# LeCAR-Lab/CoVO-MPC

Measured on AMD Instinct MI355X. Metric: mpc_control_steps_per_sec, higher is better.
Workload: dtype f32; 1 GPU; covo-online tracking_zigzag N=65536 H=32 lam=0.01 sigma=0.5 (teacher-forced on the recorded inputs -- noisy state, a_mean, key -- of this controller's own 300-step closed-loop episode, timed steps spread evenly over the episode; samples sharded 1x65536, one exchange of the 516-float rank records per step: collective); controller=covo-online, task=tracking_zigzag, N_global=65536, N_local=65536, H=32, pos_stats_info=False

## Files before the change

covo_mpc_amd/csrc/sigma_ns.hip:

```cpp
#include "covo_common.hpp"
#include <cstdlib>
#include <cstring>
#include "wave_reduce.hpp"
#include "chol_lds.hpp"
#include "eps_tiles.hpp"
#include "sym_stats.hpp"
#include "noise_gemm_body.hpp"

typedef double f64x4 __attribute__((ext_vector_type(4)));

#ifdef NS_EVAL_STAMPS
#define EV_STAMP(s, i) do { if (threadIdx.x == 0) (s)[SC_STAMPS + 96 + (i)] = (double)wall_clock64(); } while (0)
#else
#define EV_STAMP(s, i) do { } while (0)
#endif
#define EV_STAMP8(s, k, i) do { if ((k) == 8) EV_STAMP(s, 70 + (i)); } while (0)
constexpr int SN = COVO_NA;
constexpr int NS_SQUARINGS = 16;
constexpr double NS_CUT_MARGIN = 1.0 / 1024.0;
constexpr double NS_SQ_TOL = 1e-7;
constexpr double NS_SQ_TGUARD = 1e10;
constexpr int NS_ITERS = 12;
constexpr double NS_TOL2 = 1e-8;
constexpr int RITZ = 4;
// ... 55 lines not shown
}

template <int MI, int MJ>
struct TileBlock {
    double a[MI][8], b[MJ][8];
};
template <int COH, class F>
__device__ __forceinline__ void tile_col_load(double (&o)[8], const double *M, int col, int kq, int hi, int kk0, int kk1, F f)
{
#pragma unroll
    for (int kk = kk0; kk < kk1; ++kk) {
        const int k = 32 * kq + 4 * kk + hi;
        o[kk] = f(gld<COH>(M + (size_t)k * SN + col), k, col);
    }
}
template <int COH, int MI, int MJ, class F>
__device__ __forceinline__ void block_load(TileBlock<MI, MJ> &o, const double *At, const double *B, int bi, int bj, int lane, int kq, F f)
{
    const int lo = lane & 15, hi = lane >> 4;
    const int ca = 16 * MI * bi + lo, cb = 16 * MJ * bj + lo;
#pragma unroll
    for (int half = 0; half < 2; ++half) {
        tile_col_load<COH>(o.a[0], At, ca, kq, hi, 4 * half, 4 * half + 4, f);
        tile_col_load<COH>(o.b[0], B, cb, kq, hi, 4 * half, 4 * half + 4, f);
        __builtin_amdgcn_sched_barrier(0);
    }
#pragma unroll
    for (int t = 1; t < MI * MJ; ++t) {
        const int ia = t / MJ, ib = t % MJ;
        if (ib == 0) tile_col_load<COH>(o.a[ia], At, ca + 16 * ia, kq, hi, 0, 8, f);
        if (ia == 0) tile_col_load<COH>(o.b[ib], B, cb + 16 * ib, kq, hi, 0, 8, f);
        __builtin_amdgcn_sched_barrier(0);
    }
}
template <int MI, int MJ>
__device__ __forceinline__ void block_mma_reduce(const TileBlock<MI, MJ> &o, double (*red)[4][4][64], int wv, int lane, double (&v)[MI * MJ],
                                                 bool skip0 = false)
{
#pragma unroll
    for (int t = 0; t < MI * MJ; ++t) {
        if (t == 0 && skip0) continue;
        f64x4 acc = {0.0, 0.0, 0.0, 0.0};
#pragma unroll
        for (int kk = 0; kk < 8; ++kk) acc = __builtin_amdgcn_mfma_f64_16x16x4f64(o.a[t / MJ][kk], o.b[t % MJ][kk], acc, 0, 0, 0);
#pragma unroll
        for (int r = 0; r < 4; ++r) red[t][wv][r][lane] = acc[r];
        __builtin_amdgcn_sched_barrier(0);
    }
// ... 680 lines not shown
    ritz_picks<COH_NONE>(ns_xk(xb, k - 1) + (size_t)b * SN * SN, s, L);
    RitzIn in;
    ritz_load_matrix(in, Aall + (size_t)b * SN * SN, s, tid);
    ritz_load_inputs<COH_NONE>(in, s, tid);
    const double u = ritz_eval<COH_NONE>(in, ns_xk(xb, k) + (size_t)b * SN * SN, s, k, L);
    (void)ritz_decide(L, u, s, k, final, deflate);
}

__device__ __forceinline__ void ns_coef(double l, double &a, double &bq)
{
    const double rho = (l < 1.0 - 1e-9) ? 1.7320508075688772 * qm::rsq64_(1.0 + l + l * l) : 1.0;
    a = 1.5 * rho;
    bq = -0.5 * rho * rho * rho;
}

struct NsFirst {
    const double *X1, *u;
    double ya, yx, yi, yu, za, zi, zu;
    double a1, b1;
};
__device__ __forceinline__ NsFirst ns_first_setup(const double *X1, const double *s)
{
#pragma clang fp contract(off)
    NsFirst f;
    const double scale = s[SC_SCALE], delta = s[SC_DELTA], lo = s[SC_LO], gam = s[SC_GAM];
    const double alpha = s[SC_ALPHA], beta = s[SC_BETA], n0 = s[SC_N0], t1 = s[SC_SQN + 64 + 63];
    const double inv = 1.0 / scale, ib2 = 1.0 / (beta * beta), is2 = inv * inv;
    double l = sqrt(lo / scale), a0, b0;
    ns_coef(l, a0, b0);
    l = fmin(1.0, l * fma(b0 * l, l, a0));
    ns_coef(l, f.a1, f.b1);
    const double qx = n0 * ib2 * is2, qa = (2.0 * alpha * beta * ib2 + 2.0 * delta) * is2;
    const double qi = ((n0 / t1 - alpha * alpha) * ib2 + delta * delta) * is2, qu = gam * (2.0 * (1e-2 * inv) + gam);
    f.ya = fma(b0, qa, a0 * inv);
    f.yx = b0 * qx;
    f.yi = fma(b0, qi, a0 * delta * inv);
    f.yu = fma(b0, qu, a0 * gam);
    f.za = b0 * inv;
    f.zi = fma(b0, delta * inv, a0);
    f.zu = b0 * gam;
    f.X1 = X1;
    f.u = s + SC_U;
    return f;
}
struct LoadY1 {
    NsFirst f;
    __device__ __forceinline__ double operator()(double v, int r, int c) const
    {
#pragma clang fp contract(off)
        return fma(f.ya, v, fma(f.yx, f.X1[(size_t)r * SN + c], fma(f.yu * f.u[r], f.u[c], (r == c) ? f.yi : 0.0)));
    }
};
struct LoadZ1 {
    NsFirst f;
    __device__ __forceinline__ double operator()(double v, int r, int c) const
    {
#pragma clang fp contract(off)
        return fma(f.za, v, fma(f.zu * f.u[r], f.u[c], (r == c) ? f.zi : 0.0));
    }
};
template <int COH>
__device__ __forceinline__ void ns_coef_table(double *s)
{
    const double scale = s[SC_SCALE], lo = s[SC_LO];
    double l = sqrt(lo / scale);
    for (int k = 0; k < NS_ITERS; ++k) {
        double a, bq;
        ns_coef(l, a, bq);
        gst<COH>(s + SC_COEF + 2 * k, a);
        gst<COH>(s + SC_COEF + 2 * k + 1, bq);
        l = fmin(1.0, l * fma(bq * l, l, a));
    }
}

struct NsConvAsk {
// ... 6 lines not shown
    c.done = gld<COH>(s + SC_NS_DONE);
    c.e = (iter >= 2) ? gld<COH>(s + SC_ERR + (iter - 1) * 64 + lane) : 0.0;
    return c;
}
template <int COH>
__device__ __forceinline__ bool ns_converged(const NsConvAsk c, double *s, int iter, bool writer)
{
    if (c.done != 0.0) return true;
    if (iter >= 2 && wr::wave64_allsum(c.e) < NS_TOL2) {
        if (writer) gst<COH>(s + SC_NS_DONE, 1.0);
        return true;
    }
    return false;
}

__global__ __launch_bounds__(256) void ns_first_elem_kernel(const double *__restrict__ Aall, const double *__restrict__ X1all,
                                                            double *__restrict__ Yout, double *__restrict__ Ytout,
                                                            double *__restrict__ Zout, double *__restrict__ Ztout,
                                                            double *__restrict__ scall, int zbuf_out, int batch)
{
    int b, w;
    if (!ns_block(batch, b, w)) return;
    const int tid = threadIdx.x;
    double *s = scall + (size_t)b * SC_COUNT;
    if (w == 64) {
        if (tid == 0) ns_coef_table<COH_NONE>(s);
        return;
    }
    const size_t off = (size_t)b * SN * SN;
    const NsFirst f = ns_first_setup(X1all + off, s);
    if (w == 0 && tid == 0) {
        s[SC_ZBUF] = (double)zbuf_out;
        s[SC_ITERS] = 1.0;
    }
    const int ti = w >> 3, tj = w & 7;
    const int row = 16 * ti + (tid >> 4), col = 16 * tj + (tid & 15);
    const double av = Aall[off + (size_t)row * SN + col];
    store_both(Yout + off, Ytout + off, row, col, LoadY1{f}(av, row, col));
    store_both(Zout + off, Ztout + off, row, col, LoadZ1{f}(av, row, col));
}

template <int COH, int MI, int MJ>
__device__ __forceinline__ bool ns_T_block_body(const double *Y, const double *Zt, double *T, double *Tt, double *s, int iter, int w,
                                                double (*red)[4][4][64], double (*part)[4])
{
    const int tid = threadIdx.x, lane = tid & 63, wv = tid >> 6;
    constexpr int NJ = 8 / MJ;
    const int bi = w / NJ, bj = w % NJ;
    if (ns_batch_done<COH>(s, SC_NS_DONE)) return false;
    TileBlock<MI, MJ> ops;
    const NsConvAsk conv = ns_converged_ask<COH>(s, iter, lane);
    const double a = gld<COH>(s + SC_COEF + 2 * iter), bq = gld<COH>(s + SC_COEF + 2 * iter + 1);
    block_load<COH>(ops, Zt, Y, bi, bj, lane, wv, LoadPlain{});
    if (ns_converged<COH>(conv, s, iter, w == 0 && tid == 0)) return false;
// ... 131 lines not shown
    __syncthreads();
    return res;
}

__device__ __forceinline__ bool ns_persist_block(int nw, int batch, int &b, int &w, unsigned xcd0 = 0u)
{
    const unsigned slot = blockIdx.x >> 3, xcd = (blockIdx.x - xcd0) & 7u;
    b = (int)(slot / (unsigned)nw) * 8 + (int)xcd;
    w = (int)(slot % (unsigned)nw);
    return b < batch;
}
static inline dim3 ns_persist_grid(int nw, int batch) { return dim3(8 * nw * ((batch + 7) / 8)); }

struct NsBufs {
    double *Y[2], *Yt[2], *Z[2], *Zt[2], *T, *Tt;
    const double *A, *X1;
};

constexpr int NS_SQ_EVAL_WG = 8;
constexpr int NS_SQ_EVAL_WG_BATCH = 3;
template <int COH, int NEVAL>
__device__ __forceinline__ void ns_square_tail_pair_rest(const XBufs xb, double *scall, int w, unsigned xcc, double (*redp)[4][4][64],
                                                         double (*partp)[4])
{
    constexpr int NW = NS_SQ_PAIR_WG + NEVAL;
    unsigned *flags = reinterpret_cast<unsigned *>(scall + SC_FLAGS);
    unsigned phase = 1;
    for (int step = 1; step < NS_SQUARINGS; ++step) {
        if (!ns_square_pair_body<false, COH>(ns_xk(xb, step), ns_xk(xb, step + 1), scall, step, w, redp, partp)) return;
        ++phase;
        const bool gd = w == 0;
// ... 114 lines not shown
    scall += (size_t)b * SC_COUNT;
    const unsigned xcc = ns_xcc_id();
    if (w >= NS_SQ_PAIR_WG) {
        if constexpr (DYN) {
            RitzLds &L = *reinterpret_cast<RitzLds *>(dyn + 2 * 4 * 4 * 64 + 8);
            ns_square_evaluator<NEVAL, LEAN>(A + (size_t)b * SN * SN, xb, scall, w - NS_SQ_PAIR_WG, xcc, deflate, L);
        } else {
            __shared__ RitzLds L;
            ns_square_evaluator<NEVAL, LEAN>(A + (size_t)b * SN * SN, xb, scall, w - NS_SQ_PAIR_WG, xcc, deflate, L);
        }
        return;
    }
    if (w == 0) EV_STAMP(scall, 0);
    (void)ns_square_pair_body<true, COH_AGENT>(A + (size_t)b * SN * SN, ns_xk(xb, 1), scall, 0, w, redp, partp);
    int r = ns_flag_barrier<COH_AGENT>(reinterpret_cast<unsigned *>(scall + SC_FLAGS), 1u, w, NW, xcc, scall + SC_BARFAIL);
    if (r == 2 && force_agent) r = 1;
    if (w == 0 && threadIdx.x == 0) scall[SC_PROF + 5] = (double)r;
    if (r == 2) ns_square_tail_pair_rest<COH_XCD, NEVAL>(xb, scall, w, xcc, redp, partp);
    else if (r == 1) ns_square_tail_pair_rest<COH_AGENT, NEVAL>(xb, scall, w, xcc, redp, partp);
    if (w == 0) EV_STAMP(scall, 1);
}
template <int NEVAL>
__global__ __launch_bounds__(256) void ns_square_tail_pair_kernel(const double *A, const XBufs xb_all, double *scall, int batch,
                                                                  int force_agent, int deflate)
{
    ns_square_tail_pair_impl<NEVAL, false>(A, xb_all, scall, batch, force_agent, deflate);
}
__global__ __launch_bounds__(256, 3) void ns_square_tail_pair_lean_kernel(const double *A, const XBufs xb_all, double *scall, int batch,
                                                                          int force_agent, int deflate)
{
    ns_square_tail_pair_impl<NS_SQ_EVAL_WG_BATCH, true>(A, xb_all, scall, batch, force_agent, deflate);
}

constexpr int NS_PAIR_WG = 32;
template <int COH>
__device__ __forceinline__ void ns_iter_tail_pair_rest(const NsBufs &B, size_t off, double *scall, int iter_first, int w, unsigned xcc,
                                                       double (*redp)[4][4][64], double (*partp)[4], bool t_first)
{
    constexpr int iter_last = NS_ITERS - 1;
    unsigned *flags = reinterpret_cast<unsigned *>(scall + SC_FLAGS) + 64;
    unsigned phase = 1;
    for (int iter = iter_first; iter <= iter_last; ++iter) {
        const bool odd = (iter & 1) != 0;
        const double *Yi = (odd ? B.Y[1] : B.Y[0]) + off, *Yti = (odd ? B.Yt[1] : B.Yt[0]) + off;
        const double *Zi = (odd ? B.Z[1] : B.Z[0]) + off, *Zti = (odd ? B.Zt[1] : B.Zt[0]) + off;
        double *Yo = (odd ? B.Y[0] : B.Y[1]) + off, *Yto = (odd ? B.Yt[0] : B.Yt[1]) + off;
        double *Zo = (odd ? B.Z[0] : B.Z[1]) + off, *Zto = (odd ? B.Zt[0] : B.Zt[1]) + off;
        if (iter > iter_first || t_first) {
            if (!ns_T_block_body<COH, 2, 1>(Yi, Zti, B.T + off, B.Tt + off, scall, iter, w, redp, partp)) return;
            if (!ns_flag_barrier<COH>(flags, ++phase, w, NS_PAIR_WG, xcc, scall + SC_BARFAIL)) return;
        }
        (void)ns_YZ_block_body<COH, 2, 2>(Yti, Zi, B.T + off, B.Tt + off, Yo, Yto, Zo, Zto, scall, iter, odd ? 0 : 1, w, redp);
        if (iter < iter_last && !ns_flag_barrier<COH>(flags, ++phase, w, NS_PAIR_WG, xcc, scall + SC_BARFAIL)) return;
    }
}
template <int NWAVES>
__device__ void ns_logdetB_workgroup(const double *__restrict__ A, double *__restrict__ s, double *__restrict__ sm, double *__restrict__ red);
constexpr int NS_BATCH_TAIL_ITERS = 4;
__device__ __forceinline__ bool ns_wait_result(double *s)
{
    __shared__ int ready_ok;
    if (threadIdx.x == 0) {
        const long long t0 = wall_clock64();
        int good = 1;
        while (gld<COH_AGENT>(s + SC_READY) == 0.0) {
            __builtin_amdgcn_s_sleep(2);
            if (wall_clock64() - t0 > 20000000LL) {
                good = 0;
                gst<COH_AGENT>(s + SC_BARFAIL, 1.0);
                break;
            }
        }
        ready_ok = good;
    }
    __syncthreads();
    return ready_ok != 0;
}
template <bool EARLY_LOGDET>
__device__ __forceinline__ void ns_iter_tail_pair_impl(const double *A, const NsBufs B, double *scall, int batch, int force_agent, int merged,
                                                       double *ld_sm)
{
    constexpr int iter_first = EARLY_LOGDET ? 1 : NS_ITERS - NS_BATCH_TAIL_ITERS;
    double (*redp)[4][4][64] = reinterpret_cast<double (*)[4][4][64]>(ld_sm);
    __shared__ double partp[2][4];
    if (EARLY_LOGDET && blockIdx.x == 2) {
        if (merged && !ns_wait_result(scall)) return;
        ns_logdetB_workgroup<4>(A, scall, ld_sm, &partp[0][0]);
        return;
    }
    if (EARLY_LOGDET && blockIdx.x == (merged ? 3u : 1u)) {
        if (merged && !ns_wait_result(scall)) return;
        if (threadIdx.x == 0) {
            ns_coef_table<COH_AGENT>(scall);
            asm volatile("s_waitcnt vmcnt(0)" ::: "memory");
            gst<COH_AGENT>(scall + SC_BAR, 1.0);
        }
        return;
    }
    int b, w;
    if (!ns_persist_block(NS_PAIR_WG, batch, b, w, merged ? 1u : 0u)) return;
    const size_t off = (size_t)b * SN * SN;
    scall += (size_t)b * SC_COUNT;
    const unsigned xcc = ns_xcc_id();
    constexpr bool odd = (iter_first & 1) != 0;
    if (merged && !ns_wait_result(scall)) return;
    if (EARLY_LOGDET) {
        const NsFirst f = ns_first_setup(B.X1 + off, scall);
        const LoadY1 fy{f};
        const LoadZ1 fz{f};
        const int tid = threadIdx.x, lane = tid & 63, wv = tid >> 6, p = w >> 3, tj = w & 7;
        if (w == 0 && tid == 0) {
            gst<COH_AGENT>(scall + SC_ZBUF, 1.0);
            gst<COH_AGENT>(scall + SC_ITERS, 1.0);
        }
#pragma unroll
        for (int h = 0; h < 2; ++h) {
            const int row = 16 * (2 * p + h) + (lane >> 4) + 4 * wv, col = 16 * tj + (lane & 15);
            const double av = (B.A + off)[(size_t)row * SN + col];
            store_both<COH_AGENT>(B.Y[1] + off, B.Yt[1] + off, row, col, fy(av, row, col));
            store_both<COH_AGENT>(B.Z[1] + off, B.Zt[1] + off, row, col, fz(av, row, col));
        }
    } else if (!ns_T_block_body<COH_AGENT, 2, 1>((odd ? B.Y[1] : B.Y[0]) + off, (odd ? B.Zt[1] : B.Zt[0]) + off, B.T + off, B.Tt + off, scall,
                                          iter_first, w, redp, partp))
        return;
    int r = ns_flag_barrier<COH_AGENT>(reinterpret_cast<unsigned *>(scall + SC_FLAGS) + 64, 1u, w, NS_PAIR_WG, xcc, scall + SC_BARFAIL);
    if (r == 2 && force_agent) r = 1;
    if (w == 0 && threadIdx.x == 0) scall[SC_PROF + 6] = (double)r;
    if (EARLY_LOGDET) {
        __shared__ int tab_ok;
        if (threadIdx.x == 0) {
            const long long t0 = wall_clock64();
            int good = 1;
            while (gld<COH_AGENT>(scall + SC_BAR) == 0.0) {
                __builtin_amdgcn_s_sleep(1);
                if (wall_clock64() - t0 > 20000000LL) {
                    good = 0;
                    gst<COH_AGENT>(scall + SC_BARFAIL, 1.0);
                    break;
                }
            }
            tab_ok = good;
        }
        __syncthreads();
        if (!tab_ok) return;
    }
    if (r == 2) ns_iter_tail_pair_rest<COH_XCD>(B, off, scall, iter_first, w, xcc, redp, partp, EARLY_LOGDET);
    else if (r == 1) ns_iter_tail_pair_rest<COH_AGENT>(B, off, scall, iter_first, w, xcc, redp, partp, EARLY_LOGDET);
}
template <bool EARLY_LOGDET>
__global__ __launch_bounds__(256) void ns_iter_tail_pair_kernel(const double *A, const NsBufs B, double *scall, int batch, int force_agent)
{
    extern __shared__ __attribute__((aligned(16))) double ld_sm[];
    ns_iter_tail_pair_impl<EARLY_LOGDET>(A, B, scall, batch, force_agent, 0, ld_sm);
}
template <int NEVAL>
__global__ __launch_bounds__(256) void ns_chain_kernel(const double *A, const XBufs xb_all, const NsBufs B, double *scall, int force_agent,
                                                       int deflate)
{
    extern __shared__ __attribute__((aligned(16))) double ld_sm[];
    static_assert(NS_SQ_DYN_DOUBLES * sizeof(double) <= (size_t)SN * (SN + 1) * sizeof(double), "the squaring side's LDS fits the launch's");
    static_assert(NS_SQ_PAIR_WG + NEVAL <= NS_PAIR_WG, "grid = 8 x NS_PAIR_WG covers the squaring side");
    if ((blockIdx.x & 7u) == 0u) {
// ... 533 lines not shown
    double *sc = ws + (size_t)11 * batch * SN * SN;
    SymStatsOut o;
    o.rpart = sc + SC_RPART;
    o.fpart = sc + SC_FPART;
    o.diag = sc + SC_DIAG;
    o.stride = SC_COUNT;
    o.flags = sc + SC_FLAGS;
    o.ready = sc + SC_READY;
    return o;
}
const double *sigma_ns_sumlogB(void *workspace, int batch, size_t *stride_doubles)
{
    *stride_doubles = SC_COUNT;
    return reinterpret_cast<double *>(workspace) + (size_t)11 * batch * SN * SN + SC_SUMLOGB;
}
size_t sigma_ns_workspace_bytes(int batch) { return (size_t)batch * ((11 + NS_SQUARINGS - 1) * SN * SN + SC_COUNT) * sizeof(double); }

template <int MI, int MJ>
static void ns_launch_iters(hipStream_t s, const NsBufs &B, double *sc, int i_end, int batch)
{
    hipLaunchKernelGGL(ns_first_elem_kernel, ns_grid(65, batch), dim3(256), 0, s, B.A, B.X1, B.Y[1], B.Yt[1], B.Z[1], B.Zt[1], sc, 1, batch);
    for (int i = 1; i < i_end; ++i) {
        const int in = i & 1, out = in ^ 1;
        hipLaunchKernelGGL((ns_T_quad_kernel<MI, MJ>), ns_grid(64 / (MI * MJ), batch), dim3(256), 0, s, B.Y[in], B.Zt[in], B.T, B.Tt, sc, i,
                           batch);
        hipLaunchKernelGGL((ns_YZ_quad_kernel<MI, MJ>), ns_grid(128 / (MI * MJ), batch), dim3(256), 0, s, B.Yt[in], B.Z[in], B.T, B.Tt,
                           B.Y[out], B.Yt[out], B.Z[out], B.Zt[out], sc, i, out, batch);
    }
}

int launch_sigma_ns(const CovoOpts &opt, const SigmaNsDesc &d, void *workspace, hipStream_t s, const DebugMasks &dbg)
{
    const double *R = d.R;
    const int batch = d.batch;
    const float sample_sigma = d.sample_sigma;
    float *Sigma = d.Sigma;
    CovDeferred *cov = d.cov;
// ... 20 lines not shown
        COVO_CHECK_HIP(hipFuncSetAttribute(reinterpret_cast<const void *>(ns_finalize_stream_kernel),
                                           hipFuncAttributeMaxDynamicSharedMemorySize, (int)lds));
    }
    if (d.r_has_stats) A = const_cast<double *>(R);
    else hipLaunchKernelGGL(ns_prep_kernel, ns_grid(NS_TILES, batch), dim3(256), 0, s, R, A, sc, batch);
    NsBufs B;
    for (int k = 0; k < 2; ++k) {
        B.Y[k] = Y[k];
        B.Yt[k] = Yt[k];
        B.Z[k] = Z[k];
        B.Zt[k] = Zt[k];
    }
    B.T = hist0;
    B.Tt = hist0 + M;
    B.A = A;
    B.X1 = ns_xk(xb, 1);
    enum { MERGED, TWO_LAUNCH, BATCHED, PHASED } plan;
    if (!d.persistent_ok) plan = PHASED;
    else if (batch > 1) plan = BATCHED;
    else if (opt.ns_merged && d.r_has_stats && sigma_stages >= 3) plan = MERGED;
    else plan = TWO_LAUNCH;
    switch (plan) {
    case MERGED:
        hipLaunchKernelGGL((ns_chain_kernel<NS_SQ_EVAL_WG>), ns_persist_grid(NS_PAIR_WG, 1), dim3(256), lds, s, A, xb, B, sc, opt.ns_force_agent,
                           opt.ns_deflate);
        break;
    case TWO_LAUNCH:
        hipLaunchKernelGGL((ns_square_tail_pair_kernel<NS_SQ_EVAL_WG>), ns_persist_grid(NS_SQ_PAIR_WG + NS_SQ_EVAL_WG, 1), dim3(256), 0, s, A,
                           xb, sc, 1, opt.ns_force_agent, opt.ns_deflate);
        if (sigma_stages < 3) return 0;
        hipLaunchKernelGGL(ns_iter_tail_pair_kernel<true>, ns_persist_grid(NS_PAIR_WG, 1), dim3(256), lds, s, A, B, sc, 1, opt.ns_force_agent);
        break;
    case BATCHED:
        hipLaunchKernelGGL(ns_square_tail_pair_lean_kernel, ns_persist_grid(NS_SQ_PAIR_WG + NS_SQ_EVAL_WG_BATCH, batch), dim3(256), 0, s, A,
                           xb, sc, batch, opt.ns_force_agent, opt.ns_deflate);
        if (sigma_stages < 3) return 0;
        ns_launch_iters<2, 2>(s, B, sc, NS_ITERS - NS_BATCH_TAIL_ITERS, batch);
        hipLaunchKernelGGL(ns_iter_tail_pair_kernel<false>, ns_persist_grid(NS_PAIR_WG, batch), dim3(256), 4 * 4 * 4 * 64 * sizeof(double), s, A,
                           B, sc, batch, opt.ns_force_agent);
        break;
    case PHASED:
        if (batch == 1) {
            hipLaunchKernelGGL((ns_square_kernel<true, 1>), ns_grid(NS_TILES, 1), dim3(256), 0, s, A, ns_xk(xb, 1), sc, 0, 1);
            for (int i = 1; i < NS_SQUARINGS; ++i)
                hipLaunchKernelGGL((ns_square_kernel<false, 1>), ns_grid(NS_TILES, 1), dim3(256), 0, s, ns_xk(xb, i), ns_xk(xb, i + 1), sc, i, 1);
        } else {
            hipLaunchKernelGGL((ns_square_kernel<true, 2>), ns_grid(NS_SQ_PAIR_WG, batch), dim3(256), 0, s, A, ns_xk(xb, 1), sc, 0, batch);
            for (int i = 1; i < NS_SQUARINGS; ++i)
                hipLaunchKernelGGL((ns_square_kernel<false, 2>), ns_grid(NS_SQ_PAIR_WG, batch), dim3(256), 0, s, ns_xk(xb, i), ns_xk(xb, i + 1),
                                   sc, i, batch);
        }
        if (sigma_stages < 2) return 0;
        hipLaunchKernelGGL(ns_ritz_scan_kernel, dim3(batch * RITZ_NK), dim3(256), 0, s, A, xb, sc, opt.ns_deflate);
        if (sigma_stages < 3) return 0;
        if (batch == 1) ns_launch_iters<1, 1>(s, B, sc, NS_ITERS, batch);
        else ns_launch_iters<2, 2>(s, B, sc, NS_ITERS, batch);
        break;
    }
    if (sigma_stages < 4) return 0;
    const bool early_logdet = plan == MERGED || plan == TWO_LAUNCH;
    if (stream != nullptr && early_logdet) {
        const int ntiles = (stream->N + 31) / 32;
        const int workers = (ntiles - 8 + 7) / 8;
        if (ntiles >= 72 && workers <= 255) {
            hipLaunchKernelGGL(ns_finalize_stream_kernel, dim3(1 + workers), dim3(512), lds, s, Z[0], Z[1], Zt[0], Zt[1], sc, sample_sigma,
                               *stream, d.status);
            COVO_CHECK_HIP(hipGetLastError());
            if (d.streamed != nullptr) *d.streamed = true;
            return 0;
        }
    }
// ... 38 lines not shown
```

covo_mpc_amd/csrc/step_attach.hip:

```cpp
#include <cstdint>
#include <cstring>
#include "covo_common.hpp"

int check_model(const covo_env_params *p, const char *what)
{
    if (p->reward_kind != COVO_REWARD_PENYAW && p->reward_kind != COVO_REWARD_REALWORLD) {
        covo_set_error("%s: reward_kind=%d (COVO_REWARD_*)", what, p->reward_kind);
        return COVO_E_BADARG;
    }
    if (p->disturb_kind < COVO_DISTURB_NONE || p->disturb_kind > COVO_DISTURB_MIXED) {
        covo_set_error("%s: disturb_kind=%d (COVO_DISTURB_*)", what, p->disturb_kind);
        return COVO_E_BADARG;
    }
    if (covo_needs_tables(*p) && p->disturb_period <= 0) {
        covo_set_error("%s: disturb_period=%d", what, p->disturb_period);
        return COVO_E_BADARG;
    }
    return 0;
}

int check_step_attachments(const covo_ctx *h, int n_samples, int n_inst, bool sharded, int derive_keys, int mode, const float *a_cov,
                           const covo_env_params *params, const char *what, float gamma_sigma, bool fused_batch)
{
    if (sharded) {
// ... 419 lines not shown
    ++h->opt.epoch;
    return 0;
}

int covo_debug_set_ns_merged(covo_handle_t h, int on)
{
    REQUIRE(h, "covo_debug_set_ns_merged: null handle");
    h->opt.ns_merged = on ? 1 : 0;
    ++h->opt.epoch;
    return 0;
}

int covo_debug_set_ns_coherence(covo_handle_t h, int force_agent)
{
    REQUIRE(h, "covo_debug_set_ns_coherence: null handle");
    h->opt.ns_force_agent = force_agent ? 1 : 0;
    ++h->opt.epoch;
    return 0;
}

int covo_set_step_batched_staged(covo_handle_t h, int32_t on)
{
    REQUIRE(h, "covo_set_step_batched_staged: null handle");
    const int v = on ? 1 : 0;
    if (v != h->batched_staged) ++h->opt.epoch;
    h->batched_staged = v;
    return 0;
}

int covo_set_step_diag(covo_handle_t h, float *diag, int32_t n_inst)
{
// ... 257 lines not shown
```

Measured before the change: 6368 control-steps/s.

## Replace first two Newton-Schulz iterations with centered polynomial powers of A

The first two coupled Newton-Schulz iterations are collapsed into a closed-form degree-5 polynomial in a centered, scaled copy of A. Powers P2..P5 are computed with MFMA GEMM stages, and Y/Z are assembled elementwise from shifted polynomial coefficients. This removes one full iteration's T/Y/Z GEMM round and its barrier from the serial chain. In exchange it adds power-matrix kernels, five extra workspace matrices, and numerics that depend on the shift/scale conditioning. A debug bit that stops after iteration two is also added.

New measurement: 6602 control-steps/s, median of 6. 1.04x the previous value.

```diff
diff --git a/covo_mpc_amd/csrc/ns_iter2.hpp b/covo_mpc_amd/csrc/ns_iter2.hpp
--- /dev/null
+++ b/covo_mpc_amd/csrc/ns_iter2.hpp
@@ -0,0 +1,100 @@
+#pragma once
+#include <cmath>
+
+#if defined(__HIPCC__)
+#define NS2_HD __host__ __device__ __forceinline__
+#else
+#define NS2_HD inline
+#endif
+#if defined(__clang__)
+#define NS2_NOCONTRACT _Pragma("clang fp contract(off)")
+#else
+#define NS2_NOCONTRACT
+#endif
+
+struct Ns2In {
+    double a0, b0, a1, b1;
+    double p, q;
+    double yl, gam;
+};
+struct Ns2Coef {
+    double kz[5];
+    double ky[6];
+    double zu, yu;
+};
+
+NS2_HD double ns2_nu(double fro2)
+{
+    int e = 0;
+    (void)frexp(fro2, &e);
+    if (!(fro2 > 0.0) || !(fro2 < 1e300)) e = 0;
+    return ldexp(1.0, (e + 1) >> 1);
+}
+
+NS2_HD void ns2_center(double fro2, double tr, int n, double &mu, double &nu)
+{
+    NS2_NOCONTRACT
+    mu = tr / (double)n;
+    const double f2c = fro2 - tr * mu;
+    nu = ns2_nu(fmax(f2c, fro2 * 0x1p-40));
+}
+
+constexpr int ns2_binom(int k, int j)
+{
+    int r = 1;
+    for (int i = 1; i <= j; ++i) r = r * (k - j + i) / i;
+    return r;
+}
+
+NS2_HD void ns2_poly_z(const Ns2In &in, double (&c)[5])
+{
+    NS2_NOCONTRACT
+    const double a0 = in.a0, b0 = in.b0, a1 = in.a1, b1 = in.b1;
+    c[0] = a0 * a1;
+    c[1] = fma(b1, a0 * a0 * a0, a1 * b0);
+    c[2] = 3.0 * b1 * (a0 * a0 * b0);
+    c[3] = 3.0 * b1 * (a0 * b0 * b0);
+    c[4] = b1 * (b0 * b0 * b0);
+}
+
+template <int N>
+NS2_HD void ns2_shift(const double (&c)[N + 1], double p, double q, double (&kap)[N + 1])
+{
+    NS2_NOCONTRACT
+    double pj = 1.0;
+#if defined(__clang__)
+#pragma unroll
+#endif
+    for (int j = 0; j <= N; ++j) {
+        double acc = (double)ns2_binom(N, j) * c[N];
+#if defined(__clang__)
+#pragma unroll
+#endif
+        for (int k = N - 1; k >= j; --k) acc = fma(acc, q, (double)ns2_binom(k, j) * c[k]);
+        kap[j] = acc * pj;
+        pj *= p;
+    }
+}
+
+NS2_HD double ns2_horner4(const double (&c)[5], double y)
+{
+    NS2_NOCONTRACT
+    return fma(fma(fma(fma(c[4], y, c[3]), y, c[2]), y, c[1]), y, c[0]);
+}
+
+NS2_HD Ns2Coef ns2_coefs(const Ns2In &in)
+{
+    NS2_NOCONTRACT
+    Ns2Coef o;
+    double cz[5], cy[6];
+    ns2_poly_z(in, cz);
+    cy[0] = 0.0;
+    for (int k = 0; k < 5; ++k) cy[k + 1] = cz[k];
+    ns2_shift<4>(cz, in.p, in.q, o.kz);
+    ns2_shift<5>(cy, in.p, in.q, o.ky);
+    const double y1 = in.yl + in.gam, z1 = ns2_horner4(cz, y1), z0 = ns2_horner4(cz, in.yl);
+    o.zu = z1 - z0;
+    o.yu = fma(y1, z1, -(in.yl * z0));
+    if (in.gam == 0.0) o.yu = 0.0;
+    return o;
+}
diff --git a/covo_mpc_amd/csrc/sigma_ns.hip b/covo_mpc_amd/csrc/sigma_ns.hip
--- a/covo_mpc_amd/csrc/sigma_ns.hip
+++ b/covo_mpc_amd/csrc/sigma_ns.hip
@@ -6,6 +6,7 @@
 #include "eps_tiles.hpp"
 #include "sym_stats.hpp"
 #include "noise_gemm_body.hpp"
+#include "ns_iter2.hpp"
 
 typedef double f64x4 __attribute__((ext_vector_type(4)));
 
@@ -93,24 +94,30 @@
         o[kk] = f(gld<COH>(M + (size_t)k * SN + col), k, col);
     }
 }
+template <int COH, int MI, int MJ, class FA, class FB>
+__device__ __forceinline__ void block_load2(TileBlock<MI, MJ> &o, const double *At, const double *B, int bi, int bj, int lane, int kq, FA fa,
+                                            FB fb)
+{
+    const int lo = lane & 15, hi = lane >> 4;
+    const int ca = 16 * MI * bi + lo, cb = 16 * MJ * bj + lo;
+#pragma unroll
+    for (int half = 0; half < 2; ++half) {
+        tile_col_load<COH>(o.a[0], At, ca, kq, hi, 4 * half, 4 * half + 4, fa);
+        tile_col_load<COH>(o.b[0], B, cb, kq, hi, 4 * half, 4 * half + 4, fb);
+        __builtin_amdgcn_sched_barrier(0);
+    }
+#pragma unroll
+    for (int t = 1; t < MI * MJ; ++t) {
+        const int ia = t / MJ, ib = t % MJ;
+        if (ib == 0) tile_col_load<COH>(o.a[ia], At, ca + 16 * ia, kq, hi, 0, 8, fa);
+        if (ia == 0) tile_col_load<COH>(o.b[ib], B, cb + 16 * ib, kq, hi, 0, 8, fb);
+        __builtin_amdgcn_sched_barrier(0);
+    }
+}
 template <int COH, int MI, int MJ, class F>
 __device__ __forceinline__ void block_load(TileBlock<MI, MJ> &o, const double *At, const double *B, int bi, int bj, int lane, int kq, F f)
 {
-    const int lo = lane & 15, hi = lane >> 4;
-    const int ca = 16 * MI * bi + lo, cb = 16 * MJ * bj + lo;
-#pragma unroll
-    for (int half = 0; half < 2; ++half) {
-        tile_col_load<COH>(o.a[0], At, ca, kq, hi, 4 * half, 4 * half + 4, f);
-        tile_col_load<COH>(o.b[0], B, cb, kq, hi, 4 * half, 4 * half + 4, f);
-        __builtin_amdgcn_sched_barrier(0);
-    }
-#pragma unroll
-    for (int t = 1; t < MI * MJ; ++t) {
-        const int ia = t / MJ, ib = t % MJ;
-        if (ib == 0) tile_col_load<COH>(o.a[ia], At, ca + 16 * ia, kq, hi, 0, 8, f);
-        if (ia == 0) tile_col_load<COH>(o.b[ib], B, cb + 16 * ib, kq, hi, 0, 8, f);
-        __builtin_amdgcn_sched_barrier(0);
-    }
+    block_load2<COH>(o, At, B, bi, bj, lane, kq, f, f);
 }
 template <int MI, int MJ>
 __device__ __forceinline__ void block_mma_reduce(const TileBlock<MI, MJ> &o, double (*red)[4][4][64], int wv, int lane, double (&v)[MI * MJ],
@@ -821,51 +828,126 @@
     bq = -0.5 * rho * rho * rho;
 }
 
-struct NsFirst {
-    const double *X1, *u;
-    double ya, yx, yi, yu, za, zi, zu;
-    double a1, b1;
+struct NsPow {
+    double *P2, *P2t, *P3, *P4, *P5;
 };
-__device__ __forceinline__ NsFirst ns_first_setup(const double *X1, const double *s)
+__device__ __forceinline__ NsPow ns_pow_at(const NsPow &P, size_t off) { return NsPow{P.P2 + off, P.P2t + off, P.P3 + off, P.P4 + off, P.P5 + off}; }
+__device__ __forceinline__ LoadAffine ns_pow_operand(const double *s, int lane, double &nu)
 {
 #pragma clang fp contract(off)
-    NsFirst f;
+    const double tr = wr::wave64_allsum(s[SC_DIAG + lane] + s[SC_DIAG + 64 + lane]);
+    double mu;
+    ns2_center(slot_sum(s + SC_FPART, NS_TILES, lane), tr, SN, mu, nu);
+    const double inv_nu = 1.0 / nu;
+    return LoadAffine{-mu * inv_nu, -inv_nu};
+}
+template <bool SYM, bool AX, bool BX, int COH, int MI, int MJ>
+__device__ __forceinline__ void ns_pow_block_body(const double *At, const double *Bm, double *O, double *Ot, const double *s_stats, int q,
+                                                  double (*red)[4][4][64])
+{
+    const int tid = threadIdx.x, lane = tid & 63, wv = tid >> 6;
+    constexpr int NJ = 8 / MJ;
+    const int bi = q / NJ, bj = q % NJ;
+    if (SYM && MI * bi + MI - 1 < MJ * bj) return;
+    TileBlock<MI, MJ> ops;
+    block_load<COH>(ops, At, Bm, bi, bj, lane, wv, LoadPlain{});
+    if (AX || BX) {
+        double nu;
+        const LoadAffine fx = ns_pow_operand(s_stats, lane, nu);
+        const int lo = lane & 15, hi = lane >> 4;
+#pragma unroll
+        for (int kk = 0; kk < 8; ++kk) {
+            const int k = 32 * wv + 4 * kk + hi;
+#pragma unroll
+            for (int ia = 0; ia < MI; ++ia)
+                if (AX) ops.a[ia][kk] = fx(ops.a[ia][kk], k, 16 * (MI * bi + ia) + lo);
+#pragma unroll
+            for (int ib = 0; ib < MJ; ++ib)
+                if (BX) ops.b[ib][kk] = fx(ops.b[ib][kk], k, 16 * (MJ * bj + ib) + lo);
+        }
+    }
+    double v[MI * MJ];
+    block_mma_reduce(ops, red, wv, lane, v);
+#pragma unroll
+    for (int t = 0; t < MI * MJ; ++t) {
+        const int ti = MI * bi + t / MJ, tj = MJ * bj + t % MJ;
+        const int row = 16 * ti + (lane >> 4) + 4 * wv, col = 16 * tj + (lane & 15);
+        if (SYM) {
+            store_sym<COH>(O, row, col, v[t]);
+            if (Ot != nullptr) store_sym<COH>(Ot, row, col, v[t]);
+        } else {
+            gst<COH>(O + (size_t)row * SN + col, v[t]);
+            if (Ot != nullptr) gst<COH>(Ot + (size_t)col * SN + row, v[t]);
+        }
+    }
+}
+template <int COH, int MI, int MJ>
+__device__ __forceinline__ void ns_pow_stage(int stage, const double *A, const NsPow &P, const double *s_stats, int w, double (*red)[4][4][64])
+{
+    constexpr int NB = 64 / (MI * MJ);
+    if (stage == 0) ns_pow_block_body<true, true, true, COH, MI, MJ>(A, A, P.P2, P.P2t, s_stats, w, red);
+    else if (stage == 1 && w < NB) ns_pow_block_body<false, true, false, COH, MI, MJ>(A, P.P2, P.P3, nullptr, s_stats, w, red);
+    else if (stage == 1) ns_pow_block_body<true, false, false, COH, MI, MJ>(P.P2t, P.P2, P.P4, nullptr, s_stats, w - NB, red);
+    else ns_pow_block_body<false, false, false, COH, MI, MJ>(P.P2t, P.P3, P.P5, nullptr, s_stats, w, red);
+}
+template <int MI>
+constexpr int ns_pow_tri_blocks() { return (8 / MI) * (8 / MI + 1) / 2; }
+template <int MI, int MJ>
+__global__ __launch_bounds__(256) void ns_pow_kernel(const double *__restrict__ Aall, const NsPow Pall, const double *__restrict__ scall,
+                                                     int stage, int batch)
+{
+    __shared__ double red[MI * MJ][4][4][64];
+    int b, w;
+    if (!ns_block(batch, b, w)) return;
+    const size_t off = (size_t)b * SN * SN;
+    static_assert(MI == MJ, "square blocks: the triangular block map");
+    constexpr int NB = 64 / (MI * MJ), NJ = 8 / MJ;
+    if (stage == 0 || w >= NB) {
+        int bi, bj;
+        tri_tile(stage == 0 ? w : w - NB, bi, bj);
+        w = (stage == 0 ? 0 : NB) + bi * NJ + bj;
+    }
+    ns_pow_stage<COH_NONE, MI, MJ>(stage, Aall + off, ns_pow_at(Pall, off), scall + (size_t)b * SC_COUNT, w, red);
+}
+
+struct NsSecond {
+    NsPow P;
+    const double *u;
+    LoadAffine fx;
+    Ns2Coef k;
+};
+__device__ __forceinline__ NsSecond ns_second_setup(const NsPow &P, const double *s, const LoadAffine fx, double nu)
+{
+#pragma clang fp contract(off)
+    NsSecond f;
     const double scale = s[SC_SCALE], delta = s[SC_DELTA], lo = s[SC_LO], gam = s[SC_GAM];
-    const double alpha = s[SC_ALPHA], beta = s[SC_BETA], n0 = s[SC_N0], t1 = s[SC_SQN + 64 + 63];
-    const double inv = 1.0 / scale, ib2 = 1.0 / (beta * beta), is2 = inv * inv;
-    double l = sqrt(lo / scale), a0, b0;
-    ns_coef(l, a0, b0);
-    l = fmin(1.0, l * fma(b0 * l, l, a0));
-    ns_coef(l, f.a1, f.b1);
-    const double qx = n0 * ib2 * is2, qa = (2.0 * alpha * beta * ib2 + 2.0 * delta) * is2;
-    const double qi = ((n0 / t1 - alpha * alpha) * ib2 + delta * delta) * is2, qu = gam * (2.0 * (1e-2 * inv) + gam);
-    f.ya = fma(b0, qa, a0 * inv);
-    f.yx = b0 * qx;
-    f.yi = fma(b0, qi, a0 * delta * inv);
-    f.yu = fma(b0, qu, a0 * gam);
-    f.za = b0 * inv;
-    f.zi = fma(b0, delta * inv, a0);
-    f.zu = b0 * gam;
-    f.X1 = X1;
+    const double inv = 1.0 / scale, mu = -fx.alpha * nu;
+    Ns2In in;
+    double l = sqrt(lo / scale);
+    ns_coef(l, in.a0, in.b0);
+    l = fmin(1.0, l * fma(in.b0 * l, l, in.a0));
+    ns_coef(l, in.a1, in.b1);
+    in.p = nu * inv;
+    in.q = (mu + delta) * inv;
+    in.yl = 1e-2 * inv;
+    in.gam = gam;
+    f.k = ns2_coefs(in);
+    f.fx = fx;
+    f.P = P;
     f.u = s + SC_U;
     return f;
 }
-struct LoadY1 {
-    NsFirst f;
-    __device__ __forceinline__ double operator()(double v, int r, int c) const
-    {
+template <int COH>
+__device__ __forceinline__ void ns_second_elem_p5(const NsSecond &f, double av, int r, int c, double p5, double &y, double &z)
+{
 #pragma clang fp contract(off)
-        return fma(f.ya, v, fma(f.yx, f.X1[(size_t)r * SN + c], fma(f.yu * f.u[r], f.u[c], (r == c) ? f.yi : 0.0)));
-    }
-};
-struct LoadZ1 {
-    NsFirst f;
-    __device__ __forceinline__ double operator()(double v, int r, int c) const
-    {
-#pragma clang fp contract(off)
-        return fma(f.za, v, fma(f.zu * f.u[r], f.u[c], (r == c) ? f.zi : 0.0));
-    }
-};
+    const size_t i = (size_t)r * SN + c;
+    const double p2 = gld<COH>(f.P.P2 + i), p3 = gld<COH>(f.P.P3 + i), p4 = gld<COH>(f.P.P4 + i);
+    const double uu = f.u[r] * f.u[c], x = f.fx(av, r, c);
+    const bool dg = r == c;
+    z = fma(f.k.kz[1], x, fma(f.k.kz[2], p2, fma(f.k.kz[3], p3, fma(f.k.kz[4], p4, fma(f.k.zu, uu, dg ? f.k.kz[0] : 0.0)))));
+    y = fma(f.k.ky[1], x, fma(f.k.ky[2], p2, fma(f.k.ky[3], p3, fma(f.k.ky[4], p4, fma(f.k.ky[5], p5, fma(f.k.yu, uu, dg ? f.k.ky[0] : 0.0))))));
+}
 template <int COH>
 __device__ __forceinline__ void ns_coef_table(double *s)
 {
@@ -902,30 +984,53 @@
     return false;
 }
 
-__global__ __launch_bounds__(256) void ns_first_elem_kernel(const double *__restrict__ Aall, const double *__restrict__ X1all,
+template <int COH>
+__device__ __forceinline__ void ns_second_elem(const NsSecond &f, double av, int r, int c, double &y, double &z)
+{
+    ns_second_elem_p5<COH>(f, av, r, c, gld<COH>(f.P.P5 + (size_t)r * SN + c), y, z);
+}
+
+template <int MI, int MJ>
+__global__ __launch_bounds__(256) void ns_first_elem_kernel(const double *__restrict__ Aall, const NsPow Pall,
                                                             double *__restrict__ Yout, double *__restrict__ Ytout,
                                                             double *__restrict__ Zout, double *__restrict__ Ztout,
                                                             double *__restrict__ scall, int zbuf_out, int batch)
 {
+    __shared__ double red[MI * MJ][4][4][64];
+    constexpr int NB = 64 / (MI * MJ), NJ = 8 / MJ;
     int b, w;
     if (!ns_block(batch, b, w)) return;
-    const int tid = threadIdx.x;
+    const int tid = threadIdx.x, lane = tid & 63, wv = tid >> 6;
     double *s = scall + (size_t)b * SC_COUNT;
-    if (w == 64) {
+    if (w == NB) {
         if (tid == 0) ns_coef_table<COH_NONE>(s);
         return;
     }
     const size_t off = (size_t)b * SN * SN;
-    const NsFirst f = ns_first_setup(X1all + off, s);
+    const NsPow P = ns_pow_at(Pall, off);
+    const int bi = w / NJ, bj = w % NJ;
+    TileBlock<MI, MJ> ops;
+    block_load<COH_NONE>(ops, P.P2t, P.P3, bi, bj, lane, wv, LoadPlain{});
+    double nu;
+    const LoadAffine fx = ns_pow_operand(s, lane, nu);
+    const NsSecond f = ns_second_setup(P, s, fx, nu);
     if (w == 0 && tid == 0) {
         s[SC_ZBUF] = (double)zbuf_out;
-        s[SC_ITERS] = 1.0;
-    }
-    const int ti = w >> 3, tj = w & 7;
-    const int row = 16 * ti + (tid >> 4), col = 16 * tj + (tid & 15);
-    const double av = Aall[off + (size_t)row * SN + col];
-    store_both(Yout + off, Ytout + off, row, col, LoadY1{f}(av, row, col));
-    store_both(Zout + off, Ztout + off, row, col, LoadZ1{f}(av, row, col));
+        s[SC_ITERS] = 2.0;
+    }
+    if (w == 0 && tid < 64) s[SC_ERR + 64 + tid] = __builtin_inf();
+    double v[MI * MJ];
+    block_mma_reduce(ops, red, wv, lane, v);
+#pragma unroll
+    for (int t = 0; t < MI * MJ; ++t) {
+        const int ti = MI * bi + t / MJ, tj = MJ * bj + t % MJ;
+        const int row = 16 * ti + (lane >> 4) + 4 * wv, col = 16 * tj + (lane & 15);
+        P.P5[(size_t)row * SN + col] = v[t];
+        double y, z;
+        ns_second_elem_p5<COH_NONE>(f, Aall[off + (size_t)row * SN + col], row, col, v[t], y, z);
+        store_both(Yout + off, Ytout + off, row, col, y);
+        store_both(Zout + off, Ztout + off, row, col, z);
+    }
 }
 
 template <int COH, int MI, int MJ>
@@ -1087,7 +1192,8 @@
 
 struct NsBufs {
     double *Y[2], *Yt[2], *Z[2], *Zt[2], *T, *Tt;
-    const double *A, *X1;
+    const double *A;
+    NsPow P;
 };
 
 constexpr int NS_SQ_EVAL_WG = 8;
@@ -1232,7 +1338,7 @@
     if (w == 0) EV_STAMP(scall, 0);
     (void)ns_square_pair_body<true, COH_AGENT>(A + (size_t)b * SN * SN, ns_xk(xb, 1), scall, 0, w, redp, partp);
     int r = ns_flag_barrier<COH_AGENT>(reinterpret_cast<unsigned *>(scall + SC_FLAGS), 1u, w, NW, xcc, scall + SC_BARFAIL);
-    if (r == 2 && force_agent) r = 1;
+    if (r == 2 && (force_agent & 1)) r = 1;
     if (w == 0 && threadIdx.x == 0) scall[SC_PROF + 5] = (double)r;
     if (r == 2) ns_square_tail_pair_rest<COH_XCD, NEVAL>(xb, scall, w, xcc, redp, partp);
     else if (r == 1) ns_square_tail_pair_rest<COH_AGENT, NEVAL>(xb, scall, w, xcc, redp, partp);
@@ -1253,11 +1359,10 @@
 constexpr int NS_PAIR_WG = 32;
 template <int COH>
 __device__ __forceinline__ void ns_iter_tail_pair_rest(const NsBufs &B, size_t off, double *scall, int iter_first, int w, unsigned xcc,
-                                                       double (*redp)[4][4][64], double (*partp)[4], bool t_first)
+                                                       double (*redp)[4][4][64], double (*partp)[4], bool t_first, unsigned phase)
 {
     constexpr int iter_last = NS_ITERS - 1;
     unsigned *flags = reinterpret_cast<unsigned *>(scall + SC_FLAGS) + 64;
-    unsigned phase = 1;
     for (int iter = iter_first; iter <= iter_last; ++iter) {
         const bool odd = (iter & 1) != 0;
         const double *Yi = (odd ? B.Y[1] : B.Y[0]) + off, *Yti = (odd ? B.Yt[1] : B.Yt[0]) + off;
@@ -1274,6 +1379,59 @@
 }
 template <int NWAVES>
 __device__ void ns_logdetB_workgroup(const double *__restrict__ A, double *__restrict__ s, double *__restrict__ sm, double *__restrict__ red);
+__device__ __forceinline__ bool ns_wait_result(double *s);
+template <int COH>
+__device__ __forceinline__ void ns_iter_tail_all(const NsBufs &B, const NsPow &P, size_t off, double *scall, const LoadAffine fx, double nu,
+                                                 int merged, int stop2, int w,
+                                                 unsigned xcc, double (*redp)[4][4][64], double (*partp)[4])
+{
+    unsigned *flags = reinterpret_cast<unsigned *>(scall + SC_FLAGS) + 64;
+    const int tid = threadIdx.x, lane = tid & 63, wv = tid >> 6;
+    ns_pow_stage<COH, 2, 2>(1, B.A + off, P, scall, w, redp);
+    if (!ns_flag_barrier<COH>(flags, 2u, w, NS_PAIR_WG, xcc, scall + SC_BARFAIL)) return;
+    ns_pow_stage<COH, 2, 1>(2, B.A + off, P, scall, w, redp);
+    if (!ns_flag_barrier<COH>(flags, 3u, w, NS_PAIR_WG, xcc, scall + SC_BARFAIL)) return;
+    if (w == 0) EV_STAMP(scall, 94);
+    if (merged && !ns_wait_result(scall)) return;
+    if (w == 0) EV_STAMP(scall, 95);
+    {
+        const NsSecond f = ns_second_setup(P, scall, fx, nu);
+        const int p = w >> 3, tj = w & 7;
+        if (w == 0 && tid == 0) {
+            gst<COH_AGENT>(scall + SC_ZBUF, 0.0);
+            gst<COH_AGENT>(scall + SC_ITERS, 2.0);
+        }
+        if (w == 0 && tid < 64) gst<COH>(scall + SC_ERR + 64 + tid, __builtin_inf());
+#pragma unroll
+        for (int h = 0; h < 2; ++h) {
+            const int row = 16 * (2 * p + h) + (lane >> 4) + 4 * wv, col = 16 * tj + (lane & 15);
+            double y, z;
+            ns_second_elem<COH>(f, (B.A + off)[(size_t)row * SN + col], row, col, y, z);
+            store_both<COH>(B.Y[0] + off, B.Yt[0] + off, row, col, y);
+            store_both<COH>(B.Z[0] + off, B.Zt[0] + off, row, col, z);
+        }
+    }
+    if (!ns_flag_barrier<COH>(flags, 4u, w, NS_PAIR_WG, xcc, scall + SC_BARFAIL)) return;
+    if (w == 0 && tid == 0) scall[SC_PROF + 6] = (COH == COH_XCD) ? 2.0 : 1.0;
+    if (stop2) return;
+    __shared__ int tab_ok;
+    if (tid == 0) {
+        const long long t0 = wall_clock64();
+        int good = 1;
+        while (gld<COH_AGENT>(scall + SC_BAR) == 0.0) {
+            __builtin_amdgcn_s_sleep(1);
+            if (wall_clock64() - t0 > 20000000LL) {
+                good = 0;
+                gst<COH_AGENT>(scall + SC_BARFAIL, 1.0);
+                break;
+            }
+        }
+        tab_ok = good;
+    }
+    __syncthreads();
+    if (!tab_ok) return;
+    ns_iter_tail_pair_rest<COH>(B, off, scall, 2, w, xcc, redp, partp, true, 4u);
+}
 constexpr int NS_BATCH_TAIL_ITERS = 4;
 __device__ __forceinline__ bool ns_wait_result(double *s)
 {
@@ -1298,7 +1456,7 @@
 __device__ __forceinline__ void ns_iter_tail_pair_impl(const double *A, const NsBufs B, double *scall, int batch, int force_agent, int merged,
                                                        double *ld_sm)
 {
-    constexpr int iter_first = EARLY_LOGDET ? 1 : NS_ITERS - NS_BATCH_TAIL_ITERS;
+    constexpr int iter_first = EARLY_LOGDET ? 2 : NS_ITERS - NS_BATCH_TAIL_ITERS;
     double (*redp)[4][4][64] = reinterpret_cast<double (*)[4][4][64]>(ld_sm);
     __shared__ double partp[2][4];
     if (EARLY_LOGDET && blockIdx.x == 2) {
@@ -1320,50 +1478,27 @@
     const size_t off = (size_t)b * SN * SN;
     scall += (size_t)b * SC_COUNT;
     const unsigned xcc = ns_xcc_id();
-    constexpr bool odd = (iter_first & 1) != 0;
-    if (merged && !ns_wait_result(scall)) return;
-    if (EARLY_LOGDET) {
-        const NsFirst f = ns_first_setup(B.X1 + off, scall);
-        const LoadY1 fy{f};
-        const LoadZ1 fz{f};
-        const int tid = threadIdx.x, lane = tid & 63, wv = tid >> 6, p = w >> 3, tj = w & 7;
-        if (w == 0 && tid == 0) {
-            gst<COH_AGENT>(scall + SC_ZBUF, 1.0);
-            gst<COH_AGENT>(scall + SC_ITERS, 1.0);
-        }
-#pragma unroll
-        for (int h = 0; h < 2; ++h) {
-            const int row = 16 * (2 * p + h) + (lane >> 4) + 4 * wv, col = 16 * tj + (lane & 15);
-            const double av = (B.A + off)[(size_t)row * SN + col];
-            store_both<COH_AGENT>(B.Y[1] + off, B.Yt[1] + off, row, col, fy(av, row, col));
-            store_both<COH_AGENT>(B.Z[1] + off, B.Zt[1] + off, row, col, fz(av, row, col));
-        }
-    } else if (!ns_T_block_body<COH_AGENT, 2, 1>((odd ? B.Y[1] : B.Y[0]) + off, (odd ? B.Zt[1] : B.Zt[0]) + off, B.T + off, B.Tt + off, scall,
-                                          iter_first, w, redp, partp))
-        return;
-    int r = ns_flag_barrier<COH_AGENT>(reinterpret_cast<unsigned *>(scall + SC_FLAGS) + 64, 1u, w, NS_PAIR_WG, xcc, scall + SC_BARFAIL);
-    if (r == 2 && force_agent) r = 1;
-    if (w == 0 && threadIdx.x == 0) scall[SC_PROF + 6] = (double)r;
-    if (EARLY_LOGDET) {
-        __shared__ int tab_ok;
-        if (threadIdx.x == 0) {
-            const long long t0 = wall_clock64();
-            int good = 1;
-            while (gld<COH_AGENT>(scall + SC_BAR) == 0.0) {
-                __builtin_amdgcn_s_sleep(1);
-                if (wall_clock64() - t0 > 20000000LL) {
-                    good = 0;
-                    gst<COH_AGENT>(scall + SC_BARFAIL, 1.0);
-                    break;
-                }
-            }
-            tab_ok = good;
-        }
-        __syncthreads();
-        if (!tab_ok) return;
-    }
-    if (r == 2) ns_iter_tail_pair_rest<COH_XCD>(B, off, scall, iter_first, w, xcc, redp, partp, EARLY_LOGDET);
-    else if (r == 1) ns_iter_tail_pair_rest<COH_AGENT>(B, off, scall, iter_first, w, xcc, redp, partp, EARLY_LOGDET);
+    unsigned *flags = reinterpret_cast<unsigned *>(scall + SC_FLAGS) + 64;
+    if constexpr (EARLY_LOGDET) {
+        const NsPow P = ns_pow_at(B.P, off);
+        ns_pow_stage<COH_AGENT, 2, 1>(0, B.A + off, P, scall, w, redp);
+        double nu;
+        const LoadAffine fx = ns_pow_operand(scall, threadIdx.x & 63, nu);
+        int r = ns_flag_barrier<COH_AGENT>(flags, 1u, w, NS_PAIR_WG, xcc, scall + SC_BARFAIL);
+        if (r == 2 && (force_agent & 1)) r = 1;
+        if (r == 2) ns_iter_tail_all<COH_XCD>(B, P, off, scall, fx, nu, merged, (force_agent >> 1) & 1, w, xcc, redp, partp);
+        else if (r == 1) ns_iter_tail_all<COH_AGENT>(B, P, off, scall, fx, nu, merged, (force_agent >> 1) & 1, w, xcc, redp, partp);
+    } else {
+        constexpr bool odd = (iter_first & 1) != 0;
+        if (!ns_T_block_body<COH_AGENT, 2, 1>((odd ? B.Y[1] : B.Y[0]) + off, (odd ? B.Zt[1] : B.Zt[0]) + off, B.T + off, B.Tt + off, scall,
+                                              iter_first, w, redp, partp))
+            return;
+        int r = ns_flag_barrier<COH_AGENT>(flags, 1u, w, NS_PAIR_WG, xcc, scall + SC_BARFAIL);
+        if (r == 2 && (force_agent & 1)) r = 1;
+        if (w == 0 && threadIdx.x == 0) scall[SC_PROF + 6] = (double)r;
+        if (r == 2) ns_iter_tail_pair_rest<COH_XCD>(B, off, scall, iter_first, w, xcc, redp, partp, false, 1u);
+        else if (r == 1) ns_iter_tail_pair_rest<COH_AGENT>(B, off, scall, iter_first, w, xcc, redp, partp, false, 1u);
+    }
 }
 template <bool EARLY_LOGDET>
 __global__ __launch_bounds__(256) void ns_iter_tail_pair_kernel(const double *A, const NsBufs B, double *scall, int batch, int force_agent)
@@ -1927,13 +2062,25 @@
     *stride_doubles = SC_COUNT;
     return reinterpret_cast<double *>(workspace) + (size_t)11 * batch * SN * SN + SC_SUMLOGB;
 }
-size_t sigma_ns_workspace_bytes(int batch) { return (size_t)batch * ((11 + NS_SQUARINGS - 1) * SN * SN + SC_COUNT) * sizeof(double); }
-
+constexpr int NS_WS_HIST = NS_SQUARINGS - 1, NS_WS_POW = 5;
+size_t sigma_ns_workspace_bytes(int batch)
+{
+    return (size_t)batch * ((11 + NS_WS_HIST + NS_WS_POW) * SN * SN + SC_COUNT) * sizeof(double);
+}
+
+template <int MI, int MJ>
+static void ns_launch_powers(hipStream_t s, const NsBufs &B, double *sc, int batch)
+{
+    for (int stage = 0; stage < 2; ++stage)
+        hipLaunchKernelGGL((ns_pow_kernel<MI, MJ>), ns_grid((stage == 1 ? 64 / (MI * MJ) : 0) + ns_pow_tri_blocks<MI>(), batch), dim3(256), 0,
+                           s, B.A, B.P, sc, stage, batch);
+}
 template <int MI, int MJ>
 static void ns_launch_iters(hipStream_t s, const NsBufs &B, double *sc, int i_end, int batch)
 {
-    hipLaunchKernelGGL(ns_first_elem_kernel, ns_grid(65, batch), dim3(256), 0, s, B.A, B.X1, B.Y[1], B.Yt[1], B.Z[1], B.Zt[1], sc, 1, batch);
-    for (int i = 1; i < i_end; ++i) {
+    hipLaunchKernelGGL((ns_first_elem_kernel<MI, MJ>), ns_grid(64 / (MI * MJ) + 1, batch), dim3(256), 0, s, B.A, B.P, B.Y[0], B.Yt[0], B.Z[0],
+                       B.Zt[0], sc, 0, batch);
+    for (int i = 2; i < i_end; ++i) {
         const int in = i & 1, out = in ^ 1;
         hipLaunchKernelGGL((ns_T_quad_kernel<MI, MJ>), ns_grid(64 / (MI * MJ), batch), dim3(256), 0, s, B.Y[in], B.Zt[in], B.T, B.Tt, sc, i,
                            batch);
@@ -1984,12 +2131,18 @@
     B.T = hist0;
     B.Tt = hist0 + M;
     B.A = A;
-    B.X1 = ns_xk(xb, 1);
+    double *pw = hist0 + (size_t)NS_WS_HIST * M;
+    B.P = NsPow{pw, pw + M, pw + 2 * M, pw + 3 * M, pw + 4 * M};
     enum { MERGED, TWO_LAUNCH, BATCHED, PHASED } plan;
     if (!d.persistent_ok) plan = PHASED;
     else if (batch > 1) plan = BATCHED;
     else if (opt.ns_merged && d.r_has_stats && sigma_stages >= 3) plan = MERGED;
     else plan = TWO_LAUNCH;
+    const int stop2 = (opt.ns_force_agent >> 1) & 1;
+    if ((plan == BATCHED || plan == PHASED) && sigma_stages >= 3) {
+        if (batch == 1) ns_launch_powers<1, 1>(s, B, sc, batch);
+        else ns_launch_powers<2, 2>(s, B, sc, batch);
+    }
     switch (plan) {
     case MERGED:
         hipLaunchKernelGGL((ns_chain_kernel<NS_SQ_EVAL_WG>), ns_persist_grid(NS_PAIR_WG, 1), dim3(256), lds, s, A, xb, B, sc, opt.ns_force_agent,
@@ -2005,9 +2158,10 @@
         hipLaunchKernelGGL(ns_square_tail_pair_lean_kernel, ns_persist_grid(NS_SQ_PAIR_WG + NS_SQ_EVAL_WG_BATCH, batch), dim3(256), 0, s, A,
                            xb, sc, batch, opt.ns_force_agent, opt.ns_deflate);
         if (sigma_stages < 3) return 0;
-        ns_launch_iters<2, 2>(s, B, sc, NS_ITERS - NS_BATCH_TAIL_ITERS, batch);
-        hipLaunchKernelGGL(ns_iter_tail_pair_kernel<false>, ns_persist_grid(NS_PAIR_WG, batch), dim3(256), 4 * 4 * 4 * 64 * sizeof(double), s, A,
-                           B, sc, batch, opt.ns_force_agent);
+        ns_launch_iters<2, 2>(s, B, sc, stop2 ? 2 : NS_ITERS - NS_BATCH_TAIL_ITERS, batch);
+        if (!stop2)
+            hipLaunchKernelGGL(ns_iter_tail_pair_kernel<false>, ns_persist_grid(NS_PAIR_WG, batch), dim3(256), 4 * 4 * 4 * 64 * sizeof(double), s,
+                               A, B, sc, batch, opt.ns_force_agent);
         break;
     case PHASED:
         if (batch == 1) {
@@ -2023,8 +2177,8 @@
         if (sigma_stages < 2) return 0;
         hipLaunchKernelGGL(ns_ritz_scan_kernel, dim3(batch * RITZ_NK), dim3(256), 0, s, A, xb, sc, opt.ns_deflate);
         if (sigma_stages < 3) return 0;
-        if (batch == 1) ns_launch_iters<1, 1>(s, B, sc, NS_ITERS, batch);
-        else ns_launch_iters<2, 2>(s, B, sc, NS_ITERS, batch);
+        if (batch == 1) ns_launch_iters<1, 1>(s, B, sc, stop2 ? 2 : NS_ITERS, batch);
+        else ns_launch_iters<2, 2>(s, B, sc, stop2 ? 2 : NS_ITERS, batch);
         break;
     }
     if (sigma_stages < 4) return 0;
diff --git a/covo_mpc_amd/csrc/step_attach.hip b/covo_mpc_amd/csrc/step_attach.hip
--- a/covo_mpc_amd/csrc/step_attach.hip
+++ b/covo_mpc_amd/csrc/step_attach.hip
@@ -457,7 +457,7 @@
 int covo_debug_set_ns_coherence(covo_handle_t h, int force_agent)
 {
     REQUIRE(h, "covo_debug_set_ns_coherence: null handle");
-    h->opt.ns_force_agent = force_agent ? 1 : 0;
+    h->opt.ns_force_agent = force_agent & 3;
     ++h->opt.epoch;
     return 0;
 }
```
